# lilijiangg/AutoDiffusion

Measured on AMD Instinct MI355X. Metric: images/sec (node), ADM-G ImageNet-64 4-step DDIM, higher is better.
Workload: dtype bf16

## Files before the change

autodiffusion_amd/_lib.py:

```python
from __future__ import annotations

import ctypes as C
import os

_HERE = os.path.dirname(os.path.abspath(__file__))
LIB_PATH = os.environ.get("ADM_HIP_LIB") or os.path.join(_HERE, "libadm_hip.so")
LIB_PATH_F16 = os.environ.get("ADM_HIP_LIB_F16") or os.path.join(_HERE, "libadm_hip_f16.so")
ABI_VERSION = 10


class AdmError(RuntimeError):
    pass


class StepCoefs(C.Structure):
    _fields_ = [
        ("sqrt_recip_ac", C.c_float), ("sqrt_recipm1_ac", C.c_float), ("ac", C.c_float),
        ("ac_prev", C.c_float), ("coef1", C.c_float), ("coef2", C.c_float),
        ("log_var_lo", C.c_float), ("log_var_hi", C.c_float), ("fixed_var", C.c_float),
        ("eta", C.c_float), ("nonzero", C.c_int32), ("learned_range", C.c_int32),
        ("predict_xstart", C.c_int32), ("clip_denoised", C.c_int32),
    ]


# ... 29 lines not shown
    "adm_last_error": (C.c_char_p, []),
    "adm_stream_create_cumask": (_I, [_P, _I, C.POINTER(C.c_void_p)]),
    "adm_stream_set_cus": (_I, [_P, _I]),
    "adm_stream_destroy": (_I, [_P]),
    "adm_stream_probe": (_I, [_P, _I, _P]),
    "adm_ddim_step": (_I, [_P, _P, _P, _P, _P, _P, _P, _I, _I, _I, _I, C.POINTER(StepCoefs), _P]),
    "adm_ddpm_step": (_I, [_P, _P, _P, _P, _P, _P, _P, _I, _I, _I, _I, C.POINTER(StepCoefs), _P]),
    "adm_pack_u8_nhwc": (_I, [_P, _P, _I, _I, _I, _I, _P]),
    "adm_timestep_embedding": (_I, [_P, _P, _I, _I, _F, _P]),
    "adm_linear_f32": (_I, [_P, _P, _P, _P, _P, _P, _I, _I, _I, _I, _P]),
    "adm_stem_conv3x3": (_I, [_P, _P, _P, _P, _I, _I, _I, _I, _I, _P]),
    "adm_nchw_to_nhwc_pad": (_I, [_P, _P, _I, _I, _I, _I, _I, _P]),
    "adm_gn_partial": (_I, [_P, _I, _P, _I, _P, _I, _I, _I, _P]),
    "adm_gn_finalize": (_I, [_P, _P, _P, _P, _I, _P, _P, _P, _I, _I, _I, _I, _F, _P]),
    "adm_resample": (_I, [_P, _P, _P, _P, _I, _I, _I, _I, _I, _P]),
    "adm_conv": (_I, [C.POINTER(ConvArgs), _P]),
    "adm_conv_stat_slabs": (_I, [C.POINTER(ConvArgs)]),
    "adm_conv_pick_variant": (_I, [C.POINTER(ConvArgs)]),
    "adm_gn_finalize2": (_I, [_P, _I, _I, _P, _I, _I, _P, _P, _P, _I, _P, _P, _P, _I, _I, _F, _P]),
    "adm_packed_weight_elems": (C.c_int64, [_I, _I, _I]),
    "adm_pack_conv_weight": (_I, [_P, _P, _I, _I, _I, _P]),
    "adm_packed_weight32_elems": (C.c_int64, [_I, _I, _I]),
    "adm_pack_conv_weight32": (_I, [_P, _P, _I, _I, _I, _P]),
    "adm_attention": (_I, [_P, _P, _I, _I, _I, _I, _I, _P]),
    "adm_attention_lse": (_I, [_P, _P, _P, _I, _I, _I, _I, _I, _P]),
    "adm_attention_bwd": (_I, [_P, _P, _P, _P, _P, _P, _I, _I, _I, _I, _I, _P]),
    "adm_gn_bwd_partial": (_I, [_P, _P, _P, _P, _P, _I, _I, _I, _I, _I, _I, _I, _P]),
    "adm_gn_bwd_finalize": (_I, [_P, _P, _P, _P, _I, _P, _P, _I, _I, _I, _I, _P]),
    "adm_gn_bwd_apply": (_I, [_P, _P, _P, _P, _P, _P, _P, _P, _I, _I, _I, _I, _I, _I, _I, _P]),
    "adm_grad_add": (_I, [_P, _P, _P, _I, _I, _I, _I, _I, _P]),
    "adm_logsoftmax_grad": (_I, [_P, _P, _P, _P, _I, _I, _F, _P]),
    "adm_pool_prep": (_I, [_P, _P, _P, _P, _P, _I, _I, _I, _I, _P]),
    "adm_pool_attn_fwd": (_I, [_P, _P, _P, _I, _I, _I, _I, _I, _P]),
    "adm_pool_attn_bwd": (_I, [_P, _P, _P, _P, _I, _I, _I, _I, _I, _P]),
    "adm_pool_prep_bwd": (_I, [_P, _P, _I, _I, _I, _I, _P]),
    "adm_pack_conv_weight_bwd": (_I, [_P, _P, _I, _I, _I, _P]),
    "adm_attention_cross": (_I, [_P, _I, _P, _I, _I, _P, _I, _I, _I, _I, _I, _F, _P]),
    "adm_layernorm": (_I, [_P, _P, _P, _P, C.c_int64, _I, _F, _P]),
    "adm_geglu": (_I, [_P, _P, C.c_int64, _I, _P]),
    "adm_gn_finalize_add": (_I, [_P, _P, _P, _P, _I, _P, _P, _P, _I, _I, _I, _I, _F, _P]),
    "adm_sd_step": (_I, [_P, _P, _P, _P, _P, _P, _P, _P, _P, _P, C.c_int64, C.POINTER(SdStepCoefs), _P]),
    "adm_dpm_step": (_I, [_P, _P, _P, _P, _P, _P, C.c_int64, _F, _F, _F, _F, _F, _F, _P]),
    "adm_fid_accumulate": (_I, [_P, _P, _P, _I, _I, _P]),
    "adm_conv2d": (_I, [C.POINTER(Conv2dArgs), _P]),
# ... 46 lines not shown
```

autodiffusion_amd/csrc/adm_backward.hip:

```cpp
#include "adm_common.h"

namespace {

__device__ __forceinline__ float silu_grad(float z) {
  const float s = __builtin_amdgcn_rcpf(1.0f + __builtin_amdgcn_exp2f(z * -1.4426950408889634f));
  return s * (1.0f + z * (1.0f - s));
}

__device__ __forceinline__ long long src_pixel(int mode, int img, int y, int x, int h, int w) {
  if (mode == 0) return ((long long)img * h + y) * w + x;
  return ((long long)img * (h / 2) + y / 2) * (w / 2) + x / 2;
}

__global__ void __launch_bounds__(256)
gn_bwd_partial_kernel(const uint16_t* __restrict__ x, const uint16_t* __restrict__ dy, const float* __restrict__ aa,
                      const float* __restrict__ ab, float* __restrict__ partial, int h, int w, int c, int slabs,
                      int silu, int dy_mode) {
  extern __shared__ __attribute__((aligned(16))) float red[];
  const int hw = h * w;
  const int groups8 = c / 8;
  const int lanes = blockDim.x / groups8;
  const int lane = threadIdx.x / groups8, g8 = threadIdx.x % groups8;
  const int slab = blockIdx.x, img = blockIdx.y;
  const int per = (hw + slabs - 1) / slabs;
  const int p_begin = slab * per, p_end = min(hw, p_begin + per);
  const float dys = dy_mode ? 0.25f : 1.0f;
  float t1[8] = {}, t2[8] = {};
  if (lane < lanes) {
    const int ch = g8 * 8;
    float a8[8], b8[8];
    *reinterpret_cast<float4*>(a8) = *reinterpret_cast<const float4*>(aa + (long long)img * c + ch);
    *reinterpret_cast<float4*>(a8 + 4) = *reinterpret_cast<const float4*>(aa + (long long)img * c + ch + 4);
    *reinterpret_cast<float4*>(b8) = *reinterpret_cast<const float4*>(ab + (long long)img * c + ch);
    *reinterpret_cast<float4*>(b8 + 4) = *reinterpret_cast<const float4*>(ab + (long long)img * c + ch + 4);
#pragma unroll 2
    for (int p = p_begin + lane; p < p_end; p += lanes) {
      const uint4 xv = *reinterpret_cast<const uint4*>(x + ((long long)img * hw + p) * c + ch);
      const uint4 gv = *reinterpret_cast<const uint4*>(dy + src_pixel(dy_mode, img, p / w, p % w, h, w) * c + ch);
      const uint32_t xu[4] = {xv.x, xv.y, xv.z, xv.w}, gu[4] = {gv.x, gv.y, gv.z, gv.w};
#pragma unroll
// ... 6 lines not shown
        }
        t1[2 * j] += g0; t2[2 * j] += g0 * x0;
        t1[2 * j + 1] += g1; t2[2 * j + 1] += g1 * x1;
      }
    }
#pragma unroll
    for (int j = 0; j < 8; ++j) {
      red[((long long)lane * c + ch + j) * 2 + 0] = t1[j];
      red[((long long)lane * c + ch + j) * 2 + 1] = t2[j];
    }
  }
  __syncthreads();
  for (int i = threadIdx.x; i < c * 2; i += blockDim.x) {
    float t = 0.0f;
    for (int l = 0; l < lanes; ++l) t += red[(long long)l * c * 2 + i];
    partial[(((long long)img * slabs + slab) * c) * 2 + i] = t;
  }
}

__global__ void __launch_bounds__(256)
gn_bwd_finalize_kernel(const float* __restrict__ partial, const float* __restrict__ aa, const float* __restrict__ stats,
                       const float* __restrict__ add, int add_stride, float* __restrict__ k1, float* __restrict__ k0, int c, int hw,
                       int slabs) {
  const int img = blockIdx.x;
  const int cpg = c / 32;
  const int grp = blockIdx.y * 8 + threadIdx.x / 32, sub = threadIdx.x % 32;
  const float mean = stats[((long long)img * 32 + grp) * 2 + 0], rstd = stats[((long long)img * 32 + grp) * 2 + 1];
  const float* pb = partial + ((long long)img * slabs * c + (long long)grp * cpg) * 2;
  const float* ab = aa + (long long)img * c + grp * cpg;
  const int items = slabs * cpg;
  double s1 = 0.0, s2 = 0.0;
  const float* eb = add ? add + (long long)img * add_stride + grp * cpg : nullptr;
  auto at = [&](int i, float2& v, float& a) {
    const int sl = i / cpg, j = i - sl * cpg;
    v = *reinterpret_cast<const float2*>(pb + ((long long)sl * c + j) * 2);
    if (eb) v.y += eb[j] * v.x;
    a = ab[j];
  };
  auto acc = [&](const float2& v, float a) {
    s1 += (double)a * (double)v.x;
    s2 += (double)a * ((double)v.y - (double)mean * (double)v.x);
  };
  int i = sub;
  for (; i + 96 < items; i += 128) {
    float2 v0, v1, v2, v3;
    float a0, a1, a2, a3;
    at(i, v0, a0); at(i + 32, v1, a1); at(i + 64, v2, a2); at(i + 96, v3, a3);
// ... 1 lines not shown
  }
  for (; i < items; i += 32) {
    float2 v;
    float a;
    at(i, v, a);
    acc(v, a);
  }
  s1 /= (double)rstd;
#pragma unroll
  for (int off = 16; off >= 1; off >>= 1) {
    s1 += __shfl_xor(s1, off);
    s2 += __shfl_xor(s2, off);
  }
  const double m = (double)cpg * (double)hw;
  const double kk1 = -(double)rstd * (double)rstd * s2 / m;
  const float f1 = (float)kk1, f0 = (float)(-(double)rstd * s1 / m - (double)mean * kk1);
  for (int j = sub; j < cpg; j += 32) {
    k1[(long long)img * c + grp * cpg + j] = f1;
    k0[(long long)img * c + grp * cpg + j] = eb ? f0 + f1 * eb[j] : f0;
  }
}

__global__ void __launch_bounds__(256)
gn_bwd_apply_kernel(const uint16_t* __restrict__ x, const uint16_t* __restrict__ dy, const float* __restrict__ aa,
                    const float* __restrict__ ab, const float* __restrict__ k1, const float* __restrict__ k0,
                    const uint16_t* __restrict__ add, uint16_t* __restrict__ out, int h, int w, int c, int slabs,
                    int silu, int dy_mode, int add_mode) {
  const int hw = h * w;
  const int groups8 = c / 8;
  const int lanes = blockDim.x / groups8;
  const int lane = threadIdx.x / groups8, g8 = threadIdx.x % groups8;
  if (lane >= lanes) return;
  const int slab = blockIdx.x, img = blockIdx.y;
  const int per = (hw + slabs - 1) / slabs;
  const int p_begin = slab * per, p_end = min(hw, p_begin + per);
  const float dys = dy_mode ? 0.25f : 1.0f, adds = add_mode ? 0.25f : 1.0f;
  const int ch = g8 * 8;
  const long long cb = (long long)img * c + ch;
  float a8[8], b8[8], k18[8], k08[8];
  *reinterpret_cast<float4*>(a8) = *reinterpret_cast<const float4*>(aa + cb);
  *reinterpret_cast<float4*>(a8 + 4) = *reinterpret_cast<const float4*>(aa + cb + 4);
  *reinterpret_cast<float4*>(k18) = *reinterpret_cast<const float4*>(k1 + cb);
  *reinterpret_cast<float4*>(k18 + 4) = *reinterpret_cast<const float4*>(k1 + cb + 4);
  *reinterpret_cast<float4*>(k08) = *reinterpret_cast<const float4*>(k0 + cb);
  *reinterpret_cast<float4*>(k08 + 4) = *reinterpret_cast<const float4*>(k0 + cb + 4);
#pragma unroll
  for (int j = 0; j < 8; ++j) b8[j] = 0.0f;
  if (silu) {
    *reinterpret_cast<float4*>(b8) = *reinterpret_cast<const float4*>(ab + cb);
    *reinterpret_cast<float4*>(b8 + 4) = *reinterpret_cast<const float4*>(ab + cb + 4);
  }
#pragma unroll 2
  for (int p = p_begin + lane; p < p_end; p += lanes) {
    const long long pix = (long long)img * hw + p;
    const int py = p / w, px = p - py * w;
    const uint4 xv = *reinterpret_cast<const uint4*>(x + pix * c + ch);
    const uint4 gv = *reinterpret_cast<const uint4*>(dy + src_pixel(dy_mode, img, py, px, h, w) * c + ch);
    uint4 av = make_uint4(0, 0, 0, 0);
    if (add) av = *reinterpret_cast<const uint4*>(add + src_pixel(add_mode, img, py, px, h, w) * c + ch);
    const uint32_t xu[4] = {xv.x, xv.y, xv.z, xv.w}, gu[4] = {gv.x, gv.y, gv.z, gv.w}, au[4] = {av.x, av.y, av.z, av.w};
// ... 1 lines not shown
#pragma unroll
    for (int j = 0; j < 8; ++j) {
      const float xx = (j & 1) ? adm_hi_f32(xu[j >> 1]) : adm_lo_f32(xu[j >> 1]);
      float gg = ((j & 1) ? adm_hi_f32(gu[j >> 1]) : adm_lo_f32(gu[j >> 1])) * dys;
      const float ad = ((j & 1) ? adm_hi_f32(au[j >> 1]) : adm_lo_f32(au[j >> 1])) * adds;
      if (silu) gg *= silu_grad(a8[j] * xx + b8[j]);
      r[j] = a8[j] * gg + k18[j] * xx + k08[j] + ad;
    }
    uint4 pk;
    pk.x = adm_pack2(r[0], r[1]);
    pk.y = adm_pack2(r[2], r[3]);
    pk.z = adm_pack2(r[4], r[5]);
    pk.w = adm_pack2(r[6], r[7]);
    *reinterpret_cast<uint4*>(out + pix * c + ch) = pk;
  }
}

__global__ void __launch_bounds__(256)
add_kernel(const uint16_t* __restrict__ a, const uint16_t* __restrict__ b, uint16_t* __restrict__ out, int n, int h,
           int w, int c, int b_mode) {
  const int cg = c / 8;
  const long long items = (long long)n * h * w * cg;
  const float bs = b_mode ? 0.25f : 1.0f;
  for (long long it = (long long)blockIdx.x * blockDim.x + threadIdx.x; it < items;
       it += (long long)gridDim.x * blockDim.x) {
    const int g = (int)(it % cg);
    const long long pix = it / cg;
    const int px = (int)(pix % w), py = (int)((pix / w) % h), img = (int)(pix / ((long long)w * h));
    const uint4 av = *reinterpret_cast<const uint4*>(a + pix * c + g * 8);
    const uint4 bv = *reinterpret_cast<const uint4*>(b + src_pixel(b_mode, img, py, px, h, w) * c + g * 8);
// ... 215 lines not shown
                                const float* k1, const float* k0, const adm_bf16* add, adm_bf16* out, int n, int h,
                                int w, int c, int silu, int dy_half, int add_half, void* stream) {
  ADM_REQUIRE(x && dy && aff_a && aff_b && k1 && k0 && out, ADM_E_ARG, "adm_gn_bwd_apply: null pointer");
  ADM_REQUIRE(n > 0 && h > 0 && w > 0 && c % 8 == 0 && c <= 2048, ADM_E_SHAPE, "adm_gn_bwd_apply: bad shape");
  ADM_REQUIRE(!(dy_half || add_half) || (h % 2 == 0 && w % 2 == 0), ADM_E_SHAPE, "adm_gn_bwd_apply: odd size with a half-resolution operand");
  ADM_REQUIRE(adm_aligned16(x) && adm_aligned16(dy) && adm_aligned16(add) && adm_aligned16(out), ADM_E_ALIGN,
              "adm_gn_bwd_apply: unaligned pointer");
  const int hw = h * w;
  const int slabs = hw >= 64 ? hw / 64 : 1;
  ADM_REQUIRE(slabs <= 65535 && n <= 65535, ADM_E_SHAPE, "adm_gn_bwd_apply: grid too large");
  hipLaunchKernelGGL(gn_bwd_apply_kernel, dim3(slabs, n), dim3(256), 0,
                     (hipStream_t)stream, x, dy, aff_a, aff_b, k1, k0, add, out, h, w, c, slabs, silu, dy_half, add_half);
  return adm_check_launch("adm_gn_bwd_apply");
}

extern "C" int adm_grad_add(const adm_bf16* a, const adm_bf16* b, adm_bf16* out, int n, int h, int w, int c, int b_half,
                            void* stream) {
  ADM_REQUIRE(a && b && out, ADM_E_ARG, "adm_grad_add: null pointer");
  ADM_REQUIRE(n > 0 && h > 0 && w > 0 && c % 8 == 0, ADM_E_SHAPE, "adm_grad_add: bad shape");
  ADM_REQUIRE(adm_aligned16(a) && adm_aligned16(b) && adm_aligned16(out), ADM_E_ALIGN, "adm_grad_add: unaligned pointer");
  hipLaunchKernelGGL(add_kernel, dim3(grid_for((long long)n * h * w * (c / 8))), dim3(256), 0, (hipStream_t)stream, a, b,
                     out, n, h, w, c, b_half);
  return adm_check_launch("adm_grad_add");
}

extern "C" int adm_logsoftmax_grad(const float* logits, const int64_t* y, float* dlogits, float* logp_sel, int n, int k,
                                   float scale, void* stream) {
  ADM_REQUIRE(logits && y && dlogits, ADM_E_ARG, "adm_logsoftmax_grad: null pointer");
  ADM_REQUIRE(n > 0 && k > 0, ADM_E_ARG, "adm_logsoftmax_grad: bad shape");
  hipLaunchKernelGGL(logsoftmax_grad_kernel, dim3(n), dim3(256), 0, (hipStream_t)stream, logits, y, dlogits, logp_sel, k, scale);
// ... 48 lines not shown
```

autodiffusion_amd/csrc/adm_norm.hip:

```cpp
#include "adm_common.h"

namespace {

__global__ void __launch_bounds__(256)
stem_kernel(const float* __restrict__ x, const float* __restrict__ w, const float* __restrict__ bias,
            uint16_t* __restrict__ out, int n, int cin, int h, int wd, int cout) {
  extern __shared__ __attribute__((aligned(16))) float sw[];
  const int kk = cin * 9;
  for (int i = threadIdx.x; i < kk * cout; i += blockDim.x) {
    const int o = i % cout, k = i / cout;
    sw[i] = w[(long long)o * kk + k];
  }
  for (int i = threadIdx.x; i < cout; i += blockDim.x) sw[kk * cout + i] = bias[i];
  __syncthreads();
  const int cg = cout / 8;
  const long long items = (long long)n * h * wd * cg;
  for (long long it = (long long)blockIdx.x * blockDim.x + threadIdx.x; it < items;
       it += (long long)gridDim.x * blockDim.x) {
    const int g = (int)(it % cg);
    const long long pix = it / cg;
    const int px = (int)(pix % wd), py = (int)((pix / wd) % h), img = (int)(pix / ((long long)wd * h));
    float acc[8];
#pragma unroll
    for (int j = 0; j < 8; ++j) acc[j] = sw[kk * cout + g * 8 + j];
// ... 201 lines not shown
      }
    }
    if (MODE == 1) {
#pragma unroll
      for (int j = 0; j < 8; ++j) acc[j] *= 0.25f;
    }
    uint4 pk;
    pk.x = adm_pack2(acc[0], acc[1]);
    pk.y = adm_pack2(acc[2], acc[3]);
    pk.z = adm_pack2(acc[4], acc[5]);
    pk.w = adm_pack2(acc[6], acc[7]);
    *reinterpret_cast<uint4*>(out + opix * c + g * 8) = pk;
  }
}

}

extern "C" int adm_stem_conv3x3(const float* x, const float* w, const float* bias, adm_bf16* out, int n, int cin,
                                int h, int wd, int cout, void* stream) {
  ADM_REQUIRE(x && w && bias && out, ADM_E_ARG, "adm_stem_conv3x3: null pointer");
  ADM_REQUIRE(n > 0 && h > 0 && wd > 0, ADM_E_ARG, "adm_stem_conv3x3: bad shape");
  ADM_REQUIRE(cin >= 1 && cin <= 8 && cout % 8 == 0 && cout <= 512, ADM_E_SHAPE,
              "adm_stem_conv3x3: cin=%d cout=%d unsupported (cin<=8, cout%%8==0, cout<=512)", cin, cout);
  ADM_REQUIRE(adm_aligned16(out), ADM_E_ALIGN, "adm_stem_conv3x3: out not 16-byte aligned");
  const size_t smem = (size_t)(cin * 9 + 1) * cout * sizeof(float);
  const long long items = (long long)n * h * wd * (cout / 8);
  int blocks = (int)((items + 255) / 256);
  if (blocks > 2048) blocks = 2048;
  hipLaunchKernelGGL(stem_kernel, dim3(blocks), dim3(256), smem, (hipStream_t)stream, x, w, bias, out, n, cin, h, wd, cout);
  return adm_check_launch("adm_stem_conv3x3");
// ... 83 lines not shown
              "adm_resample: unaligned pointer");
  const int oh = (mode == 2 || mode == 4) ? h * 2 : h / 2, ow = (mode == 2 || mode == 4) ? w * 2 : w / 2;
  const long long items = (long long)n * oh * ow * (c / 8);
  int blocks = (int)((items + 255) / 256);
  if (blocks > 4096) blocks = 4096;
  hipStream_t s = (hipStream_t)stream;
  const bool act = aff_a != nullptr;
#define LAUNCH(M, A) hipLaunchKernelGGL((resample_kernel<M, A>), dim3(blocks), dim3(256), 0, s, in, aff_a, aff_b, out, n, h, w, c)
  if (mode == 1) { if (act) LAUNCH(1, true); else LAUNCH(1, false); }
  else if (mode == 2) { if (act) LAUNCH(2, true); else LAUNCH(2, false); }
  else if (mode == 3) { if (act) LAUNCH(3, true); else LAUNCH(3, false); }
  else           LAUNCH(4, false);
#undef LAUNCH
  return adm_check_launch("adm_resample");
}
```

autodiffusion_amd/ops.py:

```python
from __future__ import annotations

import ctypes as C
import os
from typing import Optional

import torch

from . import _lib
from ._lib import AdmError, ConvArgs, StepCoefs, check

BF16 = torch.bfloat16
F16 = torch.float16


def _L(t):
    if t.dtype == BF16:
        return _lib.load()
    if t.dtype == F16:
        return _lib.load("f16")
    raise AdmError(f"expected a bfloat16 or float16 activation tensor, got {t.dtype}")
GN_EPS = 1e-5

USE_FUSED_STATS = True

# ... 142 lines not shown
        return a, b, stats
    return a, b


def resample(x, mode: str, aff=None):
    n, h, w, c = x.shape
    m = {"down": 1, "up": 2, "stride2": 3, "zero2": 4}[mode]
    oh, ow = (h * 2, w * 2) if m in (2, 4) else (h // 2, w // 2)
    out = torch.empty((n, oh, ow, c), dtype=x.dtype, device=x.device)
    a, b = aff if aff is not None else (None, None)
    check(_L(x).adm_resample(_ptr(x, x.dtype, "x"), _ptr(a, torch.float32), _ptr(b, torch.float32), _ptr(out),
                                   n, h, w, c, m, _stream()), "adm_resample")
    return out


def pack_conv_weight(w, dtype=BF16):
    cout, cin = w.shape[0], w.shape[1]
    taps = 1
    for s in w.shape[2:]:
        taps *= s
    lib = _lib.load("f16" if dtype == F16 else "bf16")
    elems = lib.adm_packed_weight_elems(cout, cin, taps)
    if elems < 0:
        raise AdmError(f"pack_conv_weight: unsupported weight shape {tuple(w.shape)} (cin % 32 == 0, taps 1|9)")
    w32 = w.detach().to(torch.float32).contiguous()
    out = torch.empty((elems,), dtype=dtype, device=w.device)
    check(lib.adm_pack_conv_weight(_ptr(w32), _ptr(out), cout, cin, taps, _stream()), "adm_pack_conv_weight")
    return out


FUSE_GN_BWD = os.environ.get("ADM_FUSE_GN_BWD", "1") != "0"
UPCONV_PHASES = os.environ.get("ADM_UPCONV_PHASES", "1") != "0"


def up_phase_weights(w):
    w32 = w.detach().to(torch.float32)
    rows = {0: [[0], [1, 2], []], 1: [[], [0, 1], [2]]}
    out = torch.zeros((4,) + tuple(w32.shape), dtype=torch.float32, device=w32.device)
    for ph in range(4):
        py, px = ph >> 1, ph & 1
        for r in range(3):
            for c in range(3):
                for ky in rows[py][r]:
                    for kx in rows[px][c]:
                        out[ph, :, :, r, c] += w32[:, :, ky, kx]
    return out
# ... 224 lines not shown
def attention_bwd(qkv, out, dout, lse, heads: int, new_order: bool):
    n, t, c3 = qkv.shape
    d = c3 // 3 // heads
    dqkv = torch.empty_like(qkv)
    delta = torch.empty((n, heads, t), dtype=torch.float32, device=qkv.device)
    check(_L(qkv).adm_attention_bwd(_ptr(qkv, qkv.dtype, "qkv"), _ptr(out, qkv.dtype, "out"), _ptr(dout, qkv.dtype, "dout"),
                                        _ptr(lse, torch.float32, "lse"), _ptr(delta), _ptr(dqkv), n, t, heads, d,
                                        int(new_order), _stream()), "adm_attention_bwd")
    return dqkv


def gn_bwd(x, dy, aff, stats, silu: bool, dy_half=False, add=None, add_half=False, partial=None, norm_add=None):
    n, h, w, c = x.shape
    hw = h * w
    lib = _L(x)
    k1 = torch.empty((n, c), dtype=torch.float32, device=x.device)
    k0 = torch.empty((n, c), dtype=torch.float32, device=x.device)
    a, b = aff
    if partial is None:
        slabs = max(1, hw // GN_BWD_SLAB_PIXELS)
        partial = torch.empty((n, slabs, c, 2), dtype=torch.float32, device=x.device)
        check(lib.adm_gn_bwd_partial(_ptr(x, x.dtype, "x"), _ptr(dy, x.dtype, "dy"), _ptr(a, torch.float32), _ptr(b, torch.float32),
                                     _ptr(partial), n, h, w, c, slabs, int(silu), int(dy_half), _stream()),
              "adm_gn_bwd_partial")
    else:
        if dy_half or tuple(partial.shape[0:1] + partial.shape[2:]) != (n, c, 2):
            raise AdmError("gn_bwd(partial=...): same-resolution dz and [n, slabs, c, 2] sums expected")
        slabs = partial.shape[1]
        silu = False
    if norm_add is not None and (norm_add.dtype != torch.float32 or norm_add.shape != (n, c) or norm_add.stride(1) != 1):
        raise AdmError("norm_add must be float32 [N, C] with unit channel stride")
    check(lib.adm_gn_bwd_finalize(_ptr(partial), _ptr(a), _ptr(stats, torch.float32, "stats"),
                                  None if norm_add is None else norm_add.data_ptr(), 0 if norm_add is None else norm_add.stride(0),
                                  _ptr(k1), _ptr(k0), n, c, hw, slabs, _stream()), "adm_gn_bwd_finalize")
    out = torch.empty_like(x)
    check(lib.adm_gn_bwd_apply(_ptr(x), _ptr(dy, x.dtype, "dy"), _ptr(a), _ptr(b), _ptr(k1), _ptr(k0), _ptr(add, x.dtype, "add"),
                               _ptr(out), n, h, w, c, int(silu), int(dy_half), int(add_half), _stream()),
          "adm_gn_bwd_apply")
    return out


def grad_add(a, b, b_half=False):
    n, h, w, c = a.shape
    out = torch.empty_like(a)
    check(_L(a).adm_grad_add(_ptr(a, a.dtype, "a"), _ptr(b, a.dtype, "b"), _ptr(out), n, h, w, c, int(b_half),
                                   _stream()), "adm_grad_add")
    return out


def logsoftmax_grad(logits, y, scale: float):
# ... 191 lines not shown
```

autodiffusion_amd/unet.py:

```python
from __future__ import annotations

from collections import OrderedDict
from typing import Dict, List, Optional, Sequence

import os

import torch

from . import ops
from ._lib import AdmError
from .arch import AttnSpec, HeadSpec, ResBlockSpec, ResampleSpec, StemSpec, UNetPlan

_ZERO_INIT_SUFFIXES = ("out_layers.3.weight", "out_layers.3.bias", "proj_out.weight", "proj_out.bias")


_warned_precision = set()


def warn_compute_dtype(what: str, flag: str):
    if flag in _warned_precision:
        return
    _warned_precision.add(flag)
    import warnings
    from . import logger
# ... 338 lines not shown
        st1 = st2 = None
        if tape is not None:
            a1, b1, st1 = ops.gn_affine(x0, d["g1"], d["b1"], x1, want_stats=True)
            aff1 = (a1, b1)
        else:
            aff1 = ops.gn_affine(x0, d["g1"], d["b1"], x1)
        virtual_up = (mode == "up" and not s.has_skip_conv and tape is None and x0.shape[1] >= 8
                      and not os.environ.get("ADM_NO_VIRTUAL_UP"))
        if virtual_up:
            assert x1 is None
            h = ops.conv(x0, d["w1"], d["c1b"], s.cout, 9, aff=aff1, silu=True, in_up=True, want_stats=True,
                         w_up=d.get("w1_up") if self.upconv_phases else None)
            xs, xs1 = x0, None
        elif mode:
            assert x1 is None
            h_in = ops.resample(x0, mode, aff1)
            xs = ops.resample(x0, mode)
            h = ops.conv(h_in, d["w1"], d["c1b"], s.cout, 9, want_stats=True)
            xs1 = None
        else:
            h = ops.conv(x0, d["w1"], d["c1b"], s.cout, 9, x1=x1, aff=aff1, silu=True, want_stats=True)
            xs, xs1 = x0, x1
        off = pr.film_off[s.prefix]
        if tape is not None:
            add2 = None
            if s.scale_shift:
                a2, b2, st2 = ops.gn_affine(h, d["g2"], d["b2"], film=film[:, off:], film_stride=pr.film_total, want_stats=True)
            else:
                add2 = film[:, off:off + s.cout]
                a2, b2, st2 = ops.gn_affine(h, d["g2"], d["b2"], add=add2, want_stats=True)
            aff2 = (a2, b2)
            tape.append(("res", s, dict(x=x0, aff1=aff1, st1=st1, h1=h, aff2=aff2, st2=st2, add2=add2)))
# ... 119 lines not shown
```

include/adm_hip.h:

```cpp
#ifndef ADM_HIP_H
#define ADM_HIP_H

#include <stdint.h>

#ifdef __cplusplus
extern "C" {
#endif

#define ADM_ABI_VERSION 10

#define ADM_E_ARG      (-1)
#define ADM_E_SHAPE    (-2)
#define ADM_E_ALIGN    (-3)

typedef uint16_t adm_bf16;

int adm_abi_version(void);
const char* adm_last_error(void);

int adm_stream_create_cumask(const uint32_t* mask, int words, void** stream_out);
int adm_stream_set_cus(void* stream, int ncu);
int adm_stream_destroy(void* stream);
int adm_stream_probe(uint32_t* out_dev, int nblocks, void* stream);

// ... 34 lines not shown
int adm_nchw_to_nhwc_pad(const float* x_nchw, adm_bf16* out_nhwc, int n, int c, int h, int w, int cpad,
                         void* stream);

int adm_gn_partial(const adm_bf16* in0, int c0, const adm_bf16* in1, int c1, float* partial,
                   int n, int hw, int slabs, void* stream);
int adm_gn_finalize(const float* partial, const float* gamma, const float* beta,
                    const float* film, int film_stride, float* aff_a, float* aff_b,
                    float* stats ,
                    int n, int c, int hw, int slabs, float eps, void* stream);
int adm_gn_finalize2(const float* partial0, int c0, int slabs0, const float* partial1, int c1, int slabs1,
                     const float* gamma, const float* beta, const float* film, int film_stride,
                     float* aff_a, float* aff_b, float* stats, int n, int hw, float eps, void* stream);

int adm_resample(const adm_bf16* in, const float* aff_a, const float* aff_b, adm_bf16* out,
                 int n, int h, int w, int c, int mode, void* stream);

typedef struct adm_conv_args {
  const adm_bf16* in0; const adm_bf16* in1;
  const adm_bf16* w_packed; const float* bias;
  const float* aff_a; const float* aff_b;
  const adm_bf16* res; void* out;
  int32_t n, h, w, c0, c1, cout;
  int32_t taps;
  int32_t prologue;
  int32_t out_mode;
  int32_t variant;
  float* out_stats;
  const adm_bf16* w_packed32;
  int32_t in_up;
  int32_t res_up;
// ... 44 lines not shown
                 float* m_out, int64_t numel, float cfg_scale, float sigma_s, float alpha_s, float a, float b0, float b1,
                 void* stream);

int adm_attention_bwd(const adm_bf16* qkv, const adm_bf16* out, const adm_bf16* dout, const float* lse,
                      float* delta_ws, adm_bf16* dqkv, int n, int t, int heads, int d, int new_order,
                      void* stream);

int adm_gn_bwd_partial(const adm_bf16* x, const adm_bf16* dy, const float* aff_a, const float* aff_b,
                       float* partial, int n, int h, int w, int c, int slabs, int silu, int dy_half,
                       void* stream);
int adm_gn_bwd_finalize(const float* partial, const float* aff_a, const float* stats, const float* add, int add_stride,
                        float* k1, float* k0, int n, int c, int hw, int slabs, void* stream);
int adm_gn_bwd_apply(const adm_bf16* x, const adm_bf16* dy, const float* aff_a, const float* aff_b,
                     const float* k1, const float* k0, const adm_bf16* add, adm_bf16* out,
                     int n, int h, int w, int c, int silu, int dy_half, int add_half, void* stream);
int adm_grad_add(const adm_bf16* a, const adm_bf16* b, adm_bf16* out, int n, int h, int w, int c,
                 int b_half, void* stream);

int adm_logsoftmax_grad(const float* logits, const int64_t* y, float* dlogits, float* logp_sel,
                        int n, int k, float scale, void* stream);

int adm_pool_prep(const adm_bf16* h, const float* aff_a, const float* aff_b, const float* pos, adm_bf16* tok,
                  int n, int hw, int c, int tpad, void* stream);
int adm_pool_attn_fwd(const adm_bf16* qkv, float* a0, float* wts, int n, int t, int tpad, int heads, int d,
                      void* stream);
int adm_pool_attn_bwd(const adm_bf16* qkv, const float* wts, const float* da0, adm_bf16* dqkv, int n, int t,
                      int tpad, int heads, int d, void* stream);
int adm_pool_prep_bwd(const adm_bf16* dtok, adm_bf16* dact, int n, int hw, int c, int tpad, void* stream);

int adm_pack_conv_weight_bwd(const float* w, adm_bf16* out, int cout, int cin, int taps, void* stream);
// ... 34 lines not shown
```

Measured before the change: 784.0.

## Fuse GroupNorm backward finalize into apply and merge downsample resample passes

Adds a fused GroupNorm-backward kernel that computes per-group coefficients in shared memory inside the apply kernel, plus a single-block path that does partial sums, finalize and apply in one launch for small spatial sizes. Also adds a resample2 kernel that produces both the GN+SiLU-activated and raw avg-pooled outputs in one pass for down blocks. The GN-backward pieces only affect backward passes, which likely do not run in DDIM sampling. The downsample fusion does run in the forward pass, saving one read of the input and one launch. The fused GN path recomputes coefficients redundantly in every slab block.

```diff
diff --git a/autodiffusion_amd/_lib.py b/autodiffusion_amd/_lib.py
--- a/autodiffusion_amd/_lib.py
+++ b/autodiffusion_amd/_lib.py
@@ -67,6 +67,7 @@
     "adm_gn_partial": (_I, [_P, _I, _P, _I, _P, _I, _I, _I, _P]),
     "adm_gn_finalize": (_I, [_P, _P, _P, _P, _I, _P, _P, _P, _I, _I, _I, _I, _F, _P]),
     "adm_resample": (_I, [_P, _P, _P, _P, _I, _I, _I, _I, _I, _P]),
+    "adm_resample2": (_I, [_P, _P, _P, _P, _P, _I, _I, _I, _I, _I, _P]),
     "adm_conv": (_I, [C.POINTER(ConvArgs), _P]),
     "adm_conv_stat_slabs": (_I, [C.POINTER(ConvArgs)]),
     "adm_conv_pick_variant": (_I, [C.POINTER(ConvArgs)]),
@@ -81,6 +82,8 @@
     "adm_gn_bwd_partial": (_I, [_P, _P, _P, _P, _P, _I, _I, _I, _I, _I, _I, _I, _P]),
     "adm_gn_bwd_finalize": (_I, [_P, _P, _P, _P, _I, _P, _P, _I, _I, _I, _I, _P]),
     "adm_gn_bwd_apply": (_I, [_P, _P, _P, _P, _P, _P, _P, _P, _I, _I, _I, _I, _I, _I, _I, _P]),
+    "adm_gn_bwd_apply_fused": (_I, [_P, _P, _P, _P, _P, _P, _P, _I, _I, _P, _P, _I, _I, _I, _I, _I, _I, _I, _P]),
+    "adm_gn_bwd_oneslab": (_I, [_P, _P, _P, _P, _P, _P, _I, _P, _P, _I, _I, _I, _I, _I, _I, _I, _P]),
     "adm_grad_add": (_I, [_P, _P, _P, _I, _I, _I, _I, _I, _P]),
     "adm_logsoftmax_grad": (_I, [_P, _P, _P, _P, _I, _I, _F, _P]),
     "adm_pool_prep": (_I, [_P, _P, _P, _P, _P, _I, _I, _I, _I, _P]),
diff --git a/autodiffusion_amd/csrc/adm_backward.hip b/autodiffusion_amd/csrc/adm_backward.hip
--- a/autodiffusion_amd/csrc/adm_backward.hip
+++ b/autodiffusion_amd/csrc/adm_backward.hip
@@ -12,18 +12,14 @@
   return ((long long)img * (h / 2) + y / 2) * (w / 2) + x / 2;
 }
 
-__global__ void __launch_bounds__(256)
-gn_bwd_partial_kernel(const uint16_t* __restrict__ x, const uint16_t* __restrict__ dy, const float* __restrict__ aa,
-                      const float* __restrict__ ab, float* __restrict__ partial, int h, int w, int c, int slabs,
-                      int silu, int dy_mode) {
-  extern __shared__ __attribute__((aligned(16))) float red[];
+__device__ __forceinline__ void gn_bwd_partial_block(const uint16_t* __restrict__ x, const uint16_t* __restrict__ dy,
+                                                     const float* __restrict__ aa, const float* __restrict__ ab, float* red,
+                                                     float* dst, int img, int p_begin, int p_end, int h, int w, int c, int silu,
+                                                     int dy_mode) {
   const int hw = h * w;
   const int groups8 = c / 8;
   const int lanes = blockDim.x / groups8;
   const int lane = threadIdx.x / groups8, g8 = threadIdx.x % groups8;
-  const int slab = blockIdx.x, img = blockIdx.y;
-  const int per = (hw + slabs - 1) / slabs;
-  const int p_begin = slab * per, p_end = min(hw, p_begin + per);
   const float dys = dy_mode ? 0.25f : 1.0f;
   float t1[8] = {}, t2[8] = {};
   if (lane < lanes) {
@@ -60,23 +56,33 @@
   for (int i = threadIdx.x; i < c * 2; i += blockDim.x) {
     float t = 0.0f;
     for (int l = 0; l < lanes; ++l) t += red[(long long)l * c * 2 + i];
-    partial[(((long long)img * slabs + slab) * c) * 2 + i] = t;
-  }
-}
-
-__global__ void __launch_bounds__(256)
-gn_bwd_finalize_kernel(const float* __restrict__ partial, const float* __restrict__ aa, const float* __restrict__ stats,
-                       const float* __restrict__ add, int add_stride, float* __restrict__ k1, float* __restrict__ k0, int c, int hw,
-                       int slabs) {
-  const int img = blockIdx.x;
+    dst[i] = t;
+  }
+}
+
+__global__ void __launch_bounds__(256)
+gn_bwd_partial_kernel(const uint16_t* __restrict__ x, const uint16_t* __restrict__ dy, const float* __restrict__ aa,
+                      const float* __restrict__ ab, float* __restrict__ partial, int h, int w, int c, int slabs,
+                      int silu, int dy_mode) {
+  extern __shared__ __attribute__((aligned(16))) float red[];
+  const int hw = h * w;
+  const int slab = blockIdx.x, img = blockIdx.y;
+  const int per = (hw + slabs - 1) / slabs;
+  const int p_begin = slab * per, p_end = min(hw, p_begin + per);
+  gn_bwd_partial_block(x, dy, aa, ab, red, partial + (((long long)img * slabs + slab) * c) * 2, img, p_begin, p_end, h, w, c,
+                       silu, dy_mode);
+}
+
+__device__ __forceinline__ void gn_bwd_group_coeffs(const float* pbase, const float* __restrict__ ab_img,
+                                                    const float* __restrict__ st, const float* __restrict__ eb_img, int c,
+                                                    int hw, int slabs, int grp, int sub, float& f1, float& f0) {
   const int cpg = c / 32;
-  const int grp = blockIdx.y * 8 + threadIdx.x / 32, sub = threadIdx.x % 32;
-  const float mean = stats[((long long)img * 32 + grp) * 2 + 0], rstd = stats[((long long)img * 32 + grp) * 2 + 1];
-  const float* pb = partial + ((long long)img * slabs * c + (long long)grp * cpg) * 2;
-  const float* ab = aa + (long long)img * c + grp * cpg;
+  const float mean = st[grp * 2 + 0], rstd = st[grp * 2 + 1];
+  const float* pb = pbase + (long long)grp * cpg * 2;
+  const float* ab = ab_img + grp * cpg;
   const int items = slabs * cpg;
   double s1 = 0.0, s2 = 0.0;
-  const float* eb = add ? add + (long long)img * add_stride + grp * cpg : nullptr;
+  const float* eb = eb_img ? eb_img + grp * cpg : nullptr;
   auto at = [&](int i, float2& v, float& a) {
     const int sl = i / cpg, j = i - sl * cpg;
     v = *reinterpret_cast<const float2*>(pb + ((long long)sl * c + j) * 2);
@@ -108,36 +114,49 @@
   }
   const double m = (double)cpg * (double)hw;
   const double kk1 = -(double)rstd * (double)rstd * s2 / m;
-  const float f1 = (float)kk1, f0 = (float)(-(double)rstd * s1 / m - (double)mean * kk1);
+  f1 = (float)kk1;
+  f0 = (float)(-(double)rstd * s1 / m - (double)mean * kk1);
+}
+
+__device__ __forceinline__ void gn_bwd_coeff_round(const float* pbase, const float* __restrict__ ab_img,
+                                                   const float* __restrict__ st, const float* __restrict__ eb_img, int c,
+                                                   int hw, int slabs, int grp0, float* k1, float* k0) {
+  const int cpg = c / 32;
+  const int grp = grp0 + threadIdx.x / 32, sub = threadIdx.x % 32;
+  float f1, f0;
+  gn_bwd_group_coeffs(pbase, ab_img, st, eb_img, c, hw, slabs, grp, sub, f1, f0);
   for (int j = sub; j < cpg; j += 32) {
-    k1[(long long)img * c + grp * cpg + j] = f1;
-    k0[(long long)img * c + grp * cpg + j] = eb ? f0 + f1 * eb[j] : f0;
-  }
-}
-
-__global__ void __launch_bounds__(256)
-gn_bwd_apply_kernel(const uint16_t* __restrict__ x, const uint16_t* __restrict__ dy, const float* __restrict__ aa,
-                    const float* __restrict__ ab, const float* __restrict__ k1, const float* __restrict__ k0,
-                    const uint16_t* __restrict__ add, uint16_t* __restrict__ out, int h, int w, int c, int slabs,
-                    int silu, int dy_mode, int add_mode) {
-  const int hw = h * w;
-  const int groups8 = c / 8;
-  const int lanes = blockDim.x / groups8;
-  const int lane = threadIdx.x / groups8, g8 = threadIdx.x % groups8;
-  if (lane >= lanes) return;
-  const int slab = blockIdx.x, img = blockIdx.y;
-  const int per = (hw + slabs - 1) / slabs;
-  const int p_begin = slab * per, p_end = min(hw, p_begin + per);
+    k1[grp * cpg + j] = f1;
+    k0[grp * cpg + j] = eb_img ? f0 + f1 * eb_img[grp * cpg + j] : f0;
+  }
+}
+
+__global__ void __launch_bounds__(256)
+gn_bwd_finalize_kernel(const float* __restrict__ partial, const float* __restrict__ aa, const float* __restrict__ stats,
+                       const float* __restrict__ add, int add_stride, float* __restrict__ k1, float* __restrict__ k0, int c, int hw,
+                       int slabs) {
+  const int img = blockIdx.x;
+  gn_bwd_coeff_round(partial + (long long)img * slabs * c * 2, aa + (long long)img * c, stats + (long long)img * 64,
+                     add ? add + (long long)img * add_stride : nullptr, c, hw, slabs, blockIdx.y * 8, k1 + (long long)img * c,
+                     k0 + (long long)img * c);
+}
+
+__device__ __forceinline__ void gn_bwd_apply_pixels(const uint16_t* __restrict__ x, const uint16_t* __restrict__ dy,
+                                                    const float* __restrict__ aa, const float* __restrict__ ab,
+                                                    const float* k1, const float* k0, const uint16_t* __restrict__ add,
+                                                    uint16_t* __restrict__ out, int img, int ch, int lane, int lanes,
+                                                    int p_begin, int p_end, int h, int w, int c, int silu, int dy_mode,
+                                                    int add_mode) {
+  const int hw = h * w;
   const float dys = dy_mode ? 0.25f : 1.0f, adds = add_mode ? 0.25f : 1.0f;
-  const int ch = g8 * 8;
   const long long cb = (long long)img * c + ch;
   float a8[8], b8[8], k18[8], k08[8];
   *reinterpret_cast<float4*>(a8) = *reinterpret_cast<const float4*>(aa + cb);
   *reinterpret_cast<float4*>(a8 + 4) = *reinterpret_cast<const float4*>(aa + cb + 4);
-  *reinterpret_cast<float4*>(k18) = *reinterpret_cast<const float4*>(k1 + cb);
-  *reinterpret_cast<float4*>(k18 + 4) = *reinterpret_cast<const float4*>(k1 + cb + 4);
-  *reinterpret_cast<float4*>(k08) = *reinterpret_cast<const float4*>(k0 + cb);
-  *reinterpret_cast<float4*>(k08 + 4) = *reinterpret_cast<const float4*>(k0 + cb + 4);
+  *reinterpret_cast<float4*>(k18) = *reinterpret_cast<const float4*>(k1 + ch);
+  *reinterpret_cast<float4*>(k18 + 4) = *reinterpret_cast<const float4*>(k1 + ch + 4);
+  *reinterpret_cast<float4*>(k08) = *reinterpret_cast<const float4*>(k0 + ch);
+  *reinterpret_cast<float4*>(k08 + 4) = *reinterpret_cast<const float4*>(k0 + ch + 4);
 #pragma unroll
   for (int j = 0; j < 8; ++j) b8[j] = 0.0f;
   if (silu) {
@@ -169,6 +188,69 @@
     pk.w = adm_pack2(r[6], r[7]);
     *reinterpret_cast<uint4*>(out + pix * c + ch) = pk;
   }
+}
+
+__global__ void __launch_bounds__(256)
+gn_bwd_apply_kernel(const uint16_t* __restrict__ x, const uint16_t* __restrict__ dy, const float* __restrict__ aa,
+                    const float* __restrict__ ab, const float* __restrict__ k1, const float* __restrict__ k0,
+                    const uint16_t* __restrict__ add, uint16_t* __restrict__ out, int h, int w, int c, int slabs,
+                    int silu, int dy_mode, int add_mode) {
+  const int hw = h * w;
+  const int groups8 = c / 8;
+  const int lanes = blockDim.x / groups8;
+  const int lane = threadIdx.x / groups8, g8 = threadIdx.x % groups8;
+  if (lane >= lanes) return;
+  const int slab = blockIdx.x, img = blockIdx.y;
+  const int per = (hw + slabs - 1) / slabs;
+  const int p_begin = slab * per, p_end = min(hw, p_begin + per);
+  gn_bwd_apply_pixels(x, dy, aa, ab, k1 + (long long)img * c, k0 + (long long)img * c, add, out, img, g8 * 8, lane, lanes,
+                      p_begin, p_end, h, w, c, silu, dy_mode, add_mode);
+}
+
+__global__ void __launch_bounds__(256)
+gn_bwd_apply_fused_kernel(const uint16_t* __restrict__ x, const uint16_t* __restrict__ dy, const float* __restrict__ aa,
+                          const float* __restrict__ ab, const float* __restrict__ partial, const float* __restrict__ stats,
+                          const float* __restrict__ norm_add, int add_stride, const uint16_t* __restrict__ add,
+                          uint16_t* __restrict__ out, int h, int w, int c, int slabs, int slabs_p, int silu, int dy_mode,
+                          int add_mode) {
+  extern __shared__ __attribute__((aligned(16))) float kk[];
+  const int hw = h * w;
+  const int slab = blockIdx.x, img = blockIdx.y;
+  for (int r = 0; r < 4; ++r)
+    gn_bwd_coeff_round(partial + (long long)img * slabs_p * c * 2, aa + (long long)img * c, stats + (long long)img * 64,
+                       norm_add ? norm_add + (long long)img * add_stride : nullptr, c, hw, slabs_p, r * 8, kk, kk + c);
+  __syncthreads();
+  const int groups8 = c / 8;
+  const int lanes = blockDim.x / groups8;
+  const int lane = threadIdx.x / groups8, g8 = threadIdx.x % groups8;
+  if (lane >= lanes) return;
+  const int per = (hw + slabs - 1) / slabs;
+  const int p_begin = slab * per, p_end = min(hw, p_begin + per);
+  gn_bwd_apply_pixels(x, dy, aa, ab, kk, kk + c, add, out, img, g8 * 8, lane, lanes, p_begin, p_end, h, w, c, silu, dy_mode,
+                      add_mode);
+}
+
+__global__ void __launch_bounds__(256)
+gn_bwd_oneslab_kernel(const uint16_t* __restrict__ x, const uint16_t* __restrict__ dy, const float* __restrict__ aa,
+                      const float* __restrict__ ab, const float* __restrict__ stats, const float* __restrict__ norm_add,
+                      int add_stride, const uint16_t* __restrict__ add, uint16_t* __restrict__ out, int h, int w, int c,
+                      int silu, int dy_mode, int add_mode) {
+  extern __shared__ __attribute__((aligned(16))) float sm[];
+  const int hw = h * w;
+  const int img = blockIdx.x;
+  const int groups8 = c / 8;
+  const int lanes = blockDim.x / groups8;
+  float* red = sm;
+  float* part = sm + (long long)lanes * c * 2;
+  gn_bwd_partial_block(x, dy, aa, ab, red, part, img, 0, hw, h, w, c, silu, dy_mode);
+  __syncthreads();
+  for (int r = 0; r < 4; ++r)
+    gn_bwd_coeff_round(part, aa + (long long)img * c, stats + (long long)img * 64,
+                       norm_add ? norm_add + (long long)img * add_stride : nullptr, c, hw, 1, r * 8, red, red + c);
+  __syncthreads();
+  const int lane = threadIdx.x / groups8, g8 = threadIdx.x % groups8;
+  if (lane >= lanes) return;
+  gn_bwd_apply_pixels(x, dy, aa, ab, red, red + c, add, out, img, g8 * 8, lane, lanes, 0, hw, h, w, c, silu, dy_mode, add_mode);
 }
 
 __global__ void __launch_bounds__(256)
@@ -414,6 +496,44 @@
   return adm_check_launch("adm_gn_bwd_apply");
 }
 
+extern "C" int adm_gn_bwd_apply_fused(const adm_bf16* x, const adm_bf16* dy, const float* aff_a, const float* aff_b,
+                                      const float* partial, const float* stats, const float* norm_add, int add_stride,
+                                      int slabs_partial, const adm_bf16* add, adm_bf16* out, int n, int h, int w, int c,
+                                      int silu, int dy_half, int add_half, void* stream) {
+  ADM_REQUIRE(x && dy && aff_a && aff_b && partial && stats && out, ADM_E_ARG, "adm_gn_bwd_apply_fused: null pointer");
+  ADM_REQUIRE(n > 0 && h > 0 && w > 0 && c % 32 == 0 && c <= 2048 && slabs_partial > 0, ADM_E_SHAPE, "adm_gn_bwd_apply_fused: bad shape");
+  ADM_REQUIRE(!(dy_half || add_half) || (h % 2 == 0 && w % 2 == 0), ADM_E_SHAPE, "adm_gn_bwd_apply_fused: odd size with a half-resolution operand");
+  ADM_REQUIRE(!norm_add || add_stride >= c, ADM_E_ARG, "adm_gn_bwd_apply_fused: add_stride < c");
+  ADM_REQUIRE(adm_aligned16(x) && adm_aligned16(dy) && adm_aligned16(add) && adm_aligned16(out), ADM_E_ALIGN,
+              "adm_gn_bwd_apply_fused: unaligned pointer");
+  const int hw = h * w;
+  int pixels = slabs_partial * 16;
+  if (pixels < 64) pixels = 64;
+  const int slabs = hw >= pixels ? hw / pixels : 1;
+  ADM_REQUIRE(slabs <= 65535 && n <= 65535, ADM_E_SHAPE, "adm_gn_bwd_apply_fused: grid too large");
+  hipLaunchKernelGGL(gn_bwd_apply_fused_kernel, dim3(slabs, n), dim3(256), (size_t)c * 2 * sizeof(float), (hipStream_t)stream,
+                     x, dy, aff_a, aff_b, partial, stats, norm_add, add_stride, add, out, h, w, c, slabs, slabs_partial, silu,
+                     dy_half, add_half);
+  return adm_check_launch("adm_gn_bwd_apply_fused");
+}
+
+extern "C" int adm_gn_bwd_oneslab(const adm_bf16* x, const adm_bf16* dy, const float* aff_a, const float* aff_b,
+                                  const float* stats, const float* norm_add, int add_stride, const adm_bf16* add,
+                                  adm_bf16* out, int n, int h, int w, int c, int silu, int dy_half, int add_half,
+                                  void* stream) {
+  ADM_REQUIRE(x && dy && aff_a && aff_b && stats && out, ADM_E_ARG, "adm_gn_bwd_oneslab: null pointer");
+  ADM_REQUIRE(n > 0 && h > 0 && w > 0 && c % 32 == 0 && c <= 2048, ADM_E_SHAPE, "adm_gn_bwd_oneslab: bad shape");
+  ADM_REQUIRE(!(dy_half || add_half) || (h % 2 == 0 && w % 2 == 0), ADM_E_SHAPE, "adm_gn_bwd_oneslab: odd size with a half-resolution operand");
+  ADM_REQUIRE(!norm_add || add_stride >= c, ADM_E_ARG, "adm_gn_bwd_oneslab: add_stride < c");
+  ADM_REQUIRE(adm_aligned16(x) && adm_aligned16(dy) && adm_aligned16(add) && adm_aligned16(out), ADM_E_ALIGN,
+              "adm_gn_bwd_oneslab: unaligned pointer");
+  const int lanes = 256 / (c / 8);
+  const size_t smem = ((size_t)lanes + 1) * c * 2 * sizeof(float);
+  hipLaunchKernelGGL(gn_bwd_oneslab_kernel, dim3(n), dim3(256), smem, (hipStream_t)stream, x, dy, aff_a, aff_b, stats,
+                     norm_add, add_stride, add, out, h, w, c, silu, dy_half, add_half);
+  return adm_check_launch("adm_gn_bwd_oneslab");
+}
+
 extern "C" int adm_grad_add(const adm_bf16* a, const adm_bf16* b, adm_bf16* out, int n, int h, int w, int c, int b_half,
                             void* stream) {
   ADM_REQUIRE(a && b && out, ADM_E_ARG, "adm_grad_add: null pointer");
diff --git a/autodiffusion_amd/csrc/adm_norm.hip b/autodiffusion_amd/csrc/adm_norm.hip
--- a/autodiffusion_amd/csrc/adm_norm.hip
+++ b/autodiffusion_amd/csrc/adm_norm.hip
@@ -239,6 +239,53 @@
   }
 }
 
+__global__ void __launch_bounds__(256)
+resample2_kernel(const uint16_t* __restrict__ in, const float* __restrict__ aff_a, const float* __restrict__ aff_b,
+                 uint16_t* __restrict__ out_act, uint16_t* __restrict__ out_raw, int n, int h, int w, int c) {
+  const int oh = h / 2, ow = w / 2;
+  const int cg = c / 8;
+  const long long items = (long long)n * oh * ow * cg;
+  for (long long it = (long long)blockIdx.x * blockDim.x + threadIdx.x; it < items;
+       it += (long long)gridDim.x * blockDim.x) {
+    const int g = (int)(it % cg);
+    const long long opix = it / cg;
+    const int ox = (int)(opix % ow), oy = (int)((opix / ow) % oh), img = (int)(opix / ((long long)ow * oh));
+    float a8[8], b8[8];
+    *reinterpret_cast<float4*>(a8) = *reinterpret_cast<const float4*>(aff_a + (long long)img * c + g * 8);
+    *reinterpret_cast<float4*>(a8 + 4) = *reinterpret_cast<const float4*>(aff_a + (long long)img * c + g * 8 + 4);
+    *reinterpret_cast<float4*>(b8) = *reinterpret_cast<const float4*>(aff_b + (long long)img * c + g * 8);
+    *reinterpret_cast<float4*>(b8 + 4) = *reinterpret_cast<const float4*>(aff_b + (long long)img * c + g * 8 + 4);
+    float act[8] = {}, raw[8] = {};
+#pragma unroll
+    for (int tp = 0; tp < 4; ++tp) {
+      const int iy = oy * 2 + tp / 2, ix = ox * 2 + tp % 2;
+      const uint4 v = *reinterpret_cast<const uint4*>(in + (((long long)img * h + iy) * w + ix) * c + g * 8);
+      const uint32_t u[4] = {v.x, v.y, v.z, v.w};
+#pragma unroll
+      for (int j = 0; j < 4; ++j) {
+        const float lo = adm_lo_f32(u[j]), hi = adm_hi_f32(u[j]);
+        raw[2 * j] += lo;
+        raw[2 * j + 1] += hi;
+        act[2 * j] += adm_silu(a8[2 * j] * lo + b8[2 * j]);
+        act[2 * j + 1] += adm_silu(a8[2 * j + 1] * hi + b8[2 * j + 1]);
+      }
+    }
+#pragma unroll
+    for (int j = 0; j < 8; ++j) { act[j] *= 0.25f; raw[j] *= 0.25f; }
+    uint4 pk;
+    pk.x = adm_pack2(act[0], act[1]);
+    pk.y = adm_pack2(act[2], act[3]);
+    pk.z = adm_pack2(act[4], act[5]);
+    pk.w = adm_pack2(act[6], act[7]);
+    *reinterpret_cast<uint4*>(out_act + opix * c + g * 8) = pk;
+    pk.x = adm_pack2(raw[0], raw[1]);
+    pk.y = adm_pack2(raw[2], raw[3]);
+    pk.z = adm_pack2(raw[4], raw[5]);
+    pk.w = adm_pack2(raw[6], raw[7]);
+    *reinterpret_cast<uint4*>(out_raw + opix * c + g * 8) = pk;
+  }
+}
+
 }
 
 extern "C" int adm_stem_conv3x3(const float* x, const float* w, const float* bias, adm_bf16* out, int n, int cin,
@@ -352,3 +399,19 @@
 #undef LAUNCH
   return adm_check_launch("adm_resample");
 }
+
+extern "C" int adm_resample2(const adm_bf16* in, const float* aff_a, const float* aff_b, adm_bf16* out_act, adm_bf16* out_raw,
+                             int n, int h, int w, int c, int mode, void* stream) {
+  ADM_REQUIRE(in && aff_a && aff_b && out_act && out_raw, ADM_E_ARG, "adm_resample2: null pointer");
+  ADM_REQUIRE(mode == 1, ADM_E_ARG, "adm_resample2: mode must be 1 (avgpool2)");
+  ADM_REQUIRE(n > 0 && h > 0 && w > 0 && c % 8 == 0, ADM_E_SHAPE, "adm_resample2: bad shape");
+  ADM_REQUIRE(h % 2 == 0 && w % 2 == 0, ADM_E_SHAPE, "adm_resample2: odd size for a 2x reduction");
+  ADM_REQUIRE(adm_aligned16(in) && adm_aligned16(out_act) && adm_aligned16(out_raw) && adm_aligned16(aff_a) && adm_aligned16(aff_b),
+              ADM_E_ALIGN, "adm_resample2: unaligned pointer");
+  const long long items = (long long)n * (h / 2) * (w / 2) * (c / 8);
+  int blocks = (int)((items + 255) / 256);
+  if (blocks > 4096) blocks = 4096;
+  hipLaunchKernelGGL(resample2_kernel, dim3(blocks), dim3(256), 0, (hipStream_t)stream, in, aff_a, aff_b, out_act, out_raw, n,
+                     h, w, c);
+  return adm_check_launch("adm_resample2");
+}
diff --git a/autodiffusion_amd/ops.py b/autodiffusion_amd/ops.py
--- a/autodiffusion_amd/ops.py
+++ b/autodiffusion_amd/ops.py
@@ -180,6 +180,18 @@
     return out
 
 
+def resample_pair(x, mode: str, aff):
+    if mode != "down":
+        raise AdmError("resample_pair: mode must be 'down'")
+    n, h, w, c = x.shape
+    out_act = torch.empty((n, h // 2, w // 2, c), dtype=x.dtype, device=x.device)
+    out_raw = torch.empty_like(out_act)
+    a, b = aff
+    check(_L(x).adm_resample2(_ptr(x, x.dtype, "x"), _ptr(a, torch.float32), _ptr(b, torch.float32), _ptr(out_act), _ptr(out_raw),
+                              n, h, w, c, 1, _stream()), "adm_resample2")
+    return out_act, out_raw
+
+
 def pack_conv_weight(w, dtype=BF16):
     cout, cin = w.shape[0], w.shape[1]
     taps = 1
@@ -196,6 +208,7 @@
 
 
 FUSE_GN_BWD = os.environ.get("ADM_FUSE_GN_BWD", "1") != "0"
+GN_BWD_SPLIT = os.environ.get("ADM_GN_BWD_SPLIT", "0") == "1"
 UPCONV_PHASES = os.environ.get("ADM_UPCONV_PHASES", "1") != "0"
 
 
@@ -450,9 +463,16 @@
     n, h, w, c = x.shape
     hw = h * w
     lib = _L(x)
-    k1 = torch.empty((n, c), dtype=torch.float32, device=x.device)
-    k0 = torch.empty((n, c), dtype=torch.float32, device=x.device)
     a, b = aff
+    if norm_add is not None and (norm_add.dtype != torch.float32 or norm_add.shape != (n, c) or norm_add.stride(1) != 1):
+        raise AdmError("norm_add must be float32 [N, C] with unit channel stride")
+    e_ptr, e_stride = (None, 0) if norm_add is None else (norm_add.data_ptr(), norm_add.stride(0))
+    if partial is None and not GN_BWD_SPLIT and hw // GN_BWD_SLAB_PIXELS <= 1:
+        out = torch.empty_like(x)
+        check(lib.adm_gn_bwd_oneslab(_ptr(x, x.dtype, "x"), _ptr(dy, x.dtype, "dy"), _ptr(a, torch.float32), _ptr(b, torch.float32),
+                                     _ptr(stats, torch.float32, "stats"), e_ptr, e_stride, _ptr(add, x.dtype, "add"), _ptr(out),
+                                     n, h, w, c, int(silu), int(dy_half), int(add_half), _stream()), "adm_gn_bwd_oneslab")
+        return out
     if partial is None:
         slabs = max(1, hw // GN_BWD_SLAB_PIXELS)
         partial = torch.empty((n, slabs, c, 2), dtype=torch.float32, device=x.device)
@@ -464,12 +484,17 @@
             raise AdmError("gn_bwd(partial=...): same-resolution dz and [n, slabs, c, 2] sums expected")
         slabs = partial.shape[1]
         silu = False
-    if norm_add is not None and (norm_add.dtype != torch.float32 or norm_add.shape != (n, c) or norm_add.stride(1) != 1):
-        raise AdmError("norm_add must be float32 [N, C] with unit channel stride")
-    check(lib.adm_gn_bwd_finalize(_ptr(partial), _ptr(a), _ptr(stats, torch.float32, "stats"),
-                                  None if norm_add is None else norm_add.data_ptr(), 0 if norm_add is None else norm_add.stride(0),
+    out = torch.empty_like(x)
+    if not GN_BWD_SPLIT:
+        check(lib.adm_gn_bwd_apply_fused(_ptr(x), _ptr(dy, x.dtype, "dy"), _ptr(a), _ptr(b), _ptr(partial),
+                                         _ptr(stats, torch.float32, "stats"), e_ptr, e_stride, slabs, _ptr(add, x.dtype, "add"),
+                                         _ptr(out), n, h, w, c, int(silu), int(dy_half), int(add_half), _stream()),
+              "adm_gn_bwd_apply_fused")
+        return out
+    k1 = torch.empty((n, c), dtype=torch.float32, device=x.device)
+    k0 = torch.empty((n, c), dtype=torch.float32, device=x.device)
+    check(lib.adm_gn_bwd_finalize(_ptr(partial), _ptr(a), _ptr(stats, torch.float32, "stats"), e_ptr, e_stride,
                                   _ptr(k1), _ptr(k0), n, c, hw, slabs, _stream()), "adm_gn_bwd_finalize")
-    out = torch.empty_like(x)
     check(lib.adm_gn_bwd_apply(_ptr(x), _ptr(dy, x.dtype, "dy"), _ptr(a), _ptr(b), _ptr(k1), _ptr(k0), _ptr(add, x.dtype, "add"),
                                _ptr(out), n, h, w, c, int(silu), int(dy_half), int(add_half), _stream()),
           "adm_gn_bwd_apply")
diff --git a/autodiffusion_amd/unet.py b/autodiffusion_amd/unet.py
--- a/autodiffusion_amd/unet.py
+++ b/autodiffusion_amd/unet.py
@@ -376,8 +376,11 @@
             xs, xs1 = x0, None
         elif mode:
             assert x1 is None
-            h_in = ops.resample(x0, mode, aff1)
-            xs = ops.resample(x0, mode)
+            if mode == "down":
+                h_in, xs = ops.resample_pair(x0, mode, aff1)
+            else:
+                h_in = ops.resample(x0, mode, aff1)
+                xs = ops.resample(x0, mode)
             h = ops.conv(h_in, d["w1"], d["c1b"], s.cout, 9, want_stats=True)
             xs1 = None
         else:
diff --git a/include/adm_hip.h b/include/adm_hip.h
--- a/include/adm_hip.h
+++ b/include/adm_hip.h
@@ -72,6 +72,8 @@
 
 int adm_resample(const adm_bf16* in, const float* aff_a, const float* aff_b, adm_bf16* out,
                  int n, int h, int w, int c, int mode, void* stream);
+int adm_resample2(const adm_bf16* in, const float* aff_a, const float* aff_b, adm_bf16* out_act, adm_bf16* out_raw,
+                  int n, int h, int w, int c, int mode, void* stream);
 
 typedef struct adm_conv_args {
   const adm_bf16* in0; const adm_bf16* in1;
@@ -146,6 +148,13 @@
 int adm_gn_bwd_apply(const adm_bf16* x, const adm_bf16* dy, const float* aff_a, const float* aff_b,
                      const float* k1, const float* k0, const adm_bf16* add, adm_bf16* out,
                      int n, int h, int w, int c, int silu, int dy_half, int add_half, void* stream);
+int adm_gn_bwd_apply_fused(const adm_bf16* x, const adm_bf16* dy, const float* aff_a, const float* aff_b,
+                           const float* partial, const float* stats, const float* norm_add, int add_stride,
+                           int slabs_partial, const adm_bf16* add, adm_bf16* out,
+                           int n, int h, int w, int c, int silu, int dy_half, int add_half, void* stream);
+int adm_gn_bwd_oneslab(const adm_bf16* x, const adm_bf16* dy, const float* aff_a, const float* aff_b,
+                       const float* stats, const float* norm_add, int add_stride, const adm_bf16* add, adm_bf16* out,
+                       int n, int h, int w, int c, int silu, int dy_half, int add_half, void* stream);
 int adm_grad_add(const adm_bf16* a, const adm_bf16* b, adm_bf16* out, int n, int h, int w, int c,
                  int b_half, void* stream);
 
```

Result: no change. 784.0 (-0.0%).
